# IONIQ6000/av1-go

Measured on AMD Instinct MI355X. Metric: encoded 4K30 frames/sec (whole node) at fixed QP; PSNR-Y delta vs libaom, higher is better.
Workload: dtype u16

## Files before the change

av1-go_amd/csrc/av1_ops32.hpp:

```cpp
#pragma once
#include "av1_ops.hpp"

namespace av1ops {

enum SlotK32 : int {
  K_SKIP = 0,
  K_PART32 = 1,
  K_PART64 = 2,
  K_USE_WIENER = 3,
  K_TXB_SKIP_Y = 4,
  K_TXB_SKIP_C = 5,
  K_EOB_Y = 8,
  K_EOB_C = 9,
  K_EOBX_Y = 10,
  K_EOBX_C = 19,
  K_DC_SIGN_Y = 26,
  K_DC_SIGN_C = 29,
  K_BASE_EOB_Y = 32,
  K_BASE_EOB_C = 36,
  K_BASE_Y = 40,
  K_BASE_C = 66,
  K_BR_Y = 92,
  K_BR_C = 113,
  K_KF_Y_MODE = 134,
  K_UV_MODE = 159,
  K_ANGLE = 172,
  K_END = 180
};
static_assert((int)K_END <= (int)S_MAX, "the slot arrays of the coder are sized by S_MAX");

constexpr BandSlots kSlots32 = { K_USE_WIENER, K_KF_Y_MODE, K_UV_MODE, K_ANGLE, K_TXB_SKIP_Y, K_TXB_SKIP_C, K_EOB_Y, K_EOB_C, K_EOBX_Y, K_EOBX_C,
                                 K_DC_SIGN_Y, K_DC_SIGN_C, K_BASE_EOB_Y, K_BASE_EOB_C, K_BASE_Y, K_BASE_C, K_BR_Y, K_BR_C, 11, 9 };

AV1_HD int slot_nsym_k32(int s) {
  if (const int n = coeff_nsym<kSlots32>(s)) return n;
  if (s == K_SKIP || s == K_USE_WIENER) return 2;
  if (s < K_KF_Y_MODE) return 10;
  if (s < K_UV_MODE) return 13;
  if (s < K_ANGLE) return 14;
  return 7;
}

template <int N> AV1_HD int scan_index32(int pos) {
  const int r = pos / N, c = pos % N, d = r + c;
  const int before = d < N ? d * (d + 1) / 2 : N * N - (2 * N - 1 - d) * (2 * N - d) / 2;
  const int rmin = imax(0, d - N + 1), rmax = imin(d, N - 1);
  return before + ((d & 1) ? r - rmin : rmax - r);
}
struct ScanTables32 { uint16_t s32[1024]; uint8_t s16[256]; };
AV1_HD void fill_scan_tables32(ScanTables32 *t, int tid = 0, int nthreads = 1) {
  for (int pos = tid; pos < 1024; pos += nthreads) t->s32[scan_index32<32>(pos)] = (uint16_t)pos;
  for (int pos = tid; pos < 256; pos += nthreads) t->s16[scan_index32<16>(pos)] = (uint8_t)pos;
}
enum { kMag32Stride = 36 };
template <int N> struct Mag32 { enum { kNibbleBytes = (N + 2) * kMag32Stride / 2, kBytes = kNibbleBytes + N * N / 8 }; };
static_assert(Mag32<32>::kBytes % 4 == 0 && Mag32<16>::kBytes % 4 == 0, "maps follow each other on dwords");
struct TokScratch32 { uint8_t *mag; const ScanTables32 *scan; };

#if defined(__HIP_DEVICE_COMPILE__)
#define AV1_SHARED_ADD(p, v) atomicAdd(p, v)
#define AV1_SHARED_MAX(p, v) atomicMax(p, v)
#else
#define AV1_SHARED_ADD(p, v) (*(p) += (v))
#define AV1_SHARED_MAX(p, v) (*(p) = *(p) > (v) ? *(p) : (v))
#endif

template <int N> struct MagMap<N, false> {
  enum { LG = N == 16 ? 4 : 5, MS = kMag32Stride };
  uint8_t *mag, *sgn;
  const ScanTables32 *scan;
  AV1_HD MagMap(const TokScratch32 &ts) : mag(ts.mag), sgn(ts.mag + Mag32<N>::kNibbleBytes), scan(ts.scan) {}
  AV1_HD int load8(const int16_t *lev, int r, int *cul) {
    struct alignas(16) L8 { int16_t v[8]; } q = *reinterpret_cast<const L8 *>(lev + 8 * r);
    unsigned packed = 0, signs = 0;
    int eob = 0, sum = 0;
    for (int j = 0; j < 8; j++) {
      const int v = q.v[j], a = iabs(v);
      if (v) eob = imax(eob, scan_index32<N>(8 * r + j) + 1);
      sum += a;
      packed |= (unsigned)(a > 15 ? 15 : a) << (4 * j);
      signs |= (unsigned)(v < 0) << j;
    }
    if (!sum) return 0;
    const int at = (((8 * r) >> LG) * MS + ((8 * r) & (N - 1))) >> 1;
    *reinterpret_cast<u16a *>(mag + at) = (uint16_t)packed;
    *reinterpret_cast<u16a *>(mag + at + 2) = (uint16_t)(packed >> 16);
    sgn[r] = (uint8_t)signs;
    *cul += sum;
    return eob;
  }
  AV1_HD int pos(int c) const { return N == 16 ? (int)scan->s16[c] : (int)scan->s32[c]; }
  AV1_HD int at(int i) const { return (mag[i >> 1] >> ((i & 1) << 2)) & 15; }
  AV1_HD int neg(int p) const { return (sgn[p >> 3] >> (p & 7)) & 1; }
};

enum { kLanes32 = 64, kBlocks32 = 4, kTile32MagBytes = kBlocks32 * (Mag32<32>::kBytes + 2 * Mag32<16>::kBytes) };
template <class T, int kStore> struct LaneVar {
  T v[kStore];
  AV1_HD T &operator[](int lane) { return v[kStore == 1 ? 0 : lane]; }
};
enum { kRoundSlots = 4 + 26 + 21, kRoundStride = 33 };
AV1_HD int round_slot(int slot, bool chroma) {
  const int be = chroma ? K_BASE_EOB_C : K_BASE_EOB_Y, ba = chroma ? K_BASE_C : K_BASE_Y, br = chroma ? K_BR_C : K_BR_Y;
  return slot >= br ? 30 + slot - br : slot >= ba ? 4 + slot - ba : slot - be;
}
AV1_HD int round_slot_global(int rs, bool chroma) {
  const int be = chroma ? K_BASE_EOB_C : K_BASE_EOB_Y, ba = chroma ? K_BASE_C : K_BASE_Y, br = chroma ? K_BR_C : K_BR_Y;
  return rs >= 30 ? br + rs - 30 : rs >= 4 ? ba + rs - 4 : be + rs;
}
struct RoundCounts { uint32_t w[kLanes32 / 4]; };

struct Tile32Mem {
  ScanTables32 scan;
  alignas(16) uint8_t mag[kTile32MagBytes];
  uint32_t round[kRoundSlots * kRoundStride];
  uint32_t run[K_END];
  int eob[kBlocks32 * 3], cul[kBlocks32 * 3];
};
AV1_HD TokScratch32 tile_scratch32(Tile32Mem &S, int b, int p) {
  return { S.mag + b * (Mag32<32>::kBytes + 2 * Mag32<16>::kBytes) + (p ? Mag32<32>::kBytes + (p - 1) * Mag32<16>::kBytes : 0), &S.scan };
}

AV1_HD int lit_words(int nbits) { return (nbits + 10) / 11; }
template <class F> AV1_HD void lit_pieces(unsigned v, int nbits, F put) {
  while (nbits > 11) { nbits -= 11; put(op_lit(11, (v >> nbits) & 0x7FFu)); }
  if (nbits > 0) put(op_lit(nbits, v & ((1u << nbits) - 1u)));
}
struct WordSink32 {
  int n;
  AV1_HD void sym(int, int) { n++; }
  AV1_HD void lit(unsigned, int nbits) { n += lit_words(nbits); }
};
struct TotalSink32 {
  uint32_t *tot; int n;
  AV1_HD void sym(int slot, int) { AV1_SHARED_ADD(&tot[slot], 1u); n++; }
  AV1_HD void split(int, int slot) { sym(slot, 0); }
  AV1_HD void lit(unsigned, int nbits) { n += lit_words(nbits); }
};
struct CountSink32 {
  uint8_t *col; bool chroma; int n;
  AV1_HD void sym(int slot, int) { col[round_slot(slot, chroma) * (kRoundStride * 4)]++; n++; }
  AV1_HD void lit(unsigned, int nbits) { n += lit_words(nbits); }
};
struct EmitSink32 {
  u16a *col; bool chroma; int n; op_t *list; uint32_t *grouped;
  AV1_HD void sym(int slot, int s) { u16a &p = col[round_slot(slot, chroma) * (kRoundStride * 2)]; grouped[p] = ((uint32_t)n << 4) | (uint32_t)s; p++; n++; }
  AV1_HD void lit(unsigned v, int nbits) { lit_pieces(v, nbits, [&](op_t o) { list[n++] = o; }); }
};
struct DirectSink32 {
  uint32_t *run; int n; op_t *list; uint32_t *grouped;
  AV1_HD void sym(int slot, int s) { grouped[run[slot]++] = ((uint32_t)n << 4) | (uint32_t)s; n++; }
  AV1_HD void split(int kind, int slot) { sym(slot, kind ? kSplitVert : kSplitHorz); }
  AV1_HD void lit(unsigned v, int nbits) { lit_pieces(v, nbits, [&](op_t o) { list[n++] = o; }); }
};

AV1_HD long block_index32(const FrameView &f, int sbr, int sbc, int b) { return (long)(sbr * 2 + (b >> 1)) * (f.w8 / 4) + sbc * 2 + (b & 1); }

template <class K> AV1_HD void tok_block32_head(const FrameView &f, K &k, int sbr, int sbc, int b, bool half) {
  const int w32 = f.w8 / 4, by = b >> 1, bx = b & 1;
  const long i = block_index32(f, sbr, sbc, b);
  if (b == 0) {
    tok_lr<kSlots32>(f, k, sbr, sbc);
    if (half) k.split(1, K_PART64);
    else k.sym(K_PART64, 3);
  }
  k.sym(K_PART32, 0);
  k.sym(K_SKIP, 0);
  tok_kf_modes<kSlots32>(k, f.y_mode[i], f.uv_mode[i], by ? f.y_mode[i - w32] : 0, bx ? f.y_mode[i - 1] : 0);
}
AV1_HD void tile_sum32(Tile32Mem &S, int b, int p, int *cul, int *dc) {
  const TokScratch32 ts = tile_scratch32(S, b, p);
  *cul = imin(S.cul[b * 3 + p], 63);
  *dc = (ts.mag[0] & 15) ? ((ts.mag[p ? (int)Mag32<16>::kNibbleBytes : (int)Mag32<32>::kNibbleBytes] & 1) ? 1 : 2) : 0;
}
struct TbCtx32 { int ac, ad, lc, ld; };
AV1_HD TbCtx32 tile_ctx32(Tile32Mem &S, int b, int p) {
  TbCtx32 c = { 0, 0, 0, 0 };
  if (b >> 1) tile_sum32(S, b - 2, p, &c.ac, &c.ad);
  if (b & 1) tile_sum32(S, b - 1, p, &c.lc, &c.ld);
  return c;
}
template <int N, class K> AV1_HD void tok_tb32_open(const FrameView &f, K &k, Tile32Mem &S, int sbr, int sbc, int b, int p, bool half) {
  if (p == 0) tok_block32_head(f, k, sbr, sbc, b, half);
  const TbCtx32 c = tile_ctx32(S, b, p);
  tok_coeffs_lead<N, kSlots32>(k, p != 0, S.eob[b * 3 + p], c.ac, c.ad, c.lc, c.ld, -1, 0);
}
AV1_HD const int16_t *tile_levels32(const FrameView &f, long i, int p) { return p == 0 ? f.lev_y + i * 1024 : (p == 1 ? f.lev_u : f.lev_v) + i * 256; }
template <int N> struct Range32 {
  enum { kRange = N * N / kLanes32 };
  AV1_HD static int count(int eob) { return (eob + kRange - 1) / kRange; }
  template <class K> AV1_HD static void pass1(K &k, Tile32Mem &S, const int16_t *lev, int b, int p, int eob, int ri) {
    const MagMap<N> M(tile_scratch32(S, b, p));
    tok_coeffs_pass1<N, kSlots32>(k, M, p != 0, lev, eob, imin(eob, (ri + 1) * kRange) - 1, ri * kRange);
  }
  template <class K> AV1_HD static void pass2(K &k, Tile32Mem &S, const int16_t *lev, int b, int p, int eob, int ri) {
    const MagMap<N> M(tile_scratch32(S, b, p));
    const TbCtx32 c = ri == 0 ? tile_ctx32(S, b, p) : TbCtx32{ 0, 0, 0, 0 };
    tok_coeffs_pass2<N, kSlots32>(k, M, p != 0, lev, c.ad, c.ld, ri * kRange, imin(eob, (ri + 1) * kRange));
  }
};

template <int N> AV1_HD void tok_tb32_total(const FrameView &f, TotalSink32 &k, Tile32Mem &S, int lane, int sbr, int sbc, int b, int p, bool half) {
  const int eob = S.eob[b * 3 + p];
  const int16_t *lev = tile_levels32(f, block_index32(f, sbr, sbc, b), p);
  if (lane == 0) tok_tb32_open<N>(f, k, S, sbr, sbc, b, p, half);
  if (lane < Range32<N>::count(eob)) { Range32<N>::pass1(k, S, lev, b, p, eob, lane); Range32<N>::pass2(k, S, lev, b, p, eob, lane); }
}

template <int N, class W>
AV1_HD int tok_tb32_emit(W &w, Tile32Mem &S, const FrameView &f, int sbr, int sbc, int b, int p, bool half, int words, op_t *list, uint32_t *grouped) {
  typedef typename W::template Var<int> LaneInt;
  typedef Range32<N> R;
  const int eob = S.eob[b * 3 + p], nr = R::count(eob);
  const int16_t *lev = tile_levels32(f, block_index32(f, sbr, sbc, b), p);
  const bool chroma = p != 0;
  LaneInt n, opened;
  if (nr <= 1) {
    w.each([&](int lane) {
      if (lane) return;
      DirectSink32 k = { S.run, words, list, grouped };
      tok_tb32_open<N>(f, k, S, sbr, sbc, b, p, half);
      if (nr) { R::pass1(k, S, lev, b, p, eob, 0); R::pass2(k, S, lev, b, p, eob, 0); }
      n[lane] = k.n;
    });
    return w.first(n);
  }
  w.each([&](int lane) {
    int c = 0, o = 0;
    if (lane == 0) {
      DirectSink32 k = { S.run, words, list, grouped };
      tok_tb32_open<N>(f, k, S, sbr, sbc, b, p, half);
      o = k.n - words;
    }
    if (lane < ((nr + 3) & ~3)) {
      uint8_t *col = reinterpret_cast<uint8_t *>(S.round) + lane;
      for (int rs = 0; rs < kRoundSlots; rs++) col[rs * (kRoundStride * 4)] = 0;
      if (lane < nr) {
        CountSink32 k = { col, chroma, 0 };
        R::pass1(k, S, lev, b, p, eob, nr - 1 - lane);
        c = k.n;
      }
    }
    opened[lane] = o; n[lane] = c + o;
  });
  const int words1 = w.scan(n);
  typename W::template Var<RoundCounts> cnt;
  const int nd = (nr + 3) >> 2;
  w.each([&](int lane) {
    if (lane >= kRoundSlots) return;
    RoundCounts &c = cnt[lane];
    AV1_UNROLL
    for (int q = 0; q < kLanes32 / 4; q++) c.w[q] = q < nd ? S.round[lane * kRoundStride + q] : 0u;
  });
  w.each([&](int lane) {
    if (lane >= kRoundSlots) return;
    const RoundCounts &c = cnt[lane];
    const int slot = round_slot_global(lane, chroma);
    uint32_t run = S.run[slot];
    AV1_UNROLL
    for (int q = 0; q < kLanes32 / 4; q++) {
      if (q >= nd) continue;
      const uint32_t u = c.w[q], p0 = run, p1 = p0 + (u & 0xFF), p2 = p1 + ((u >> 8) & 0xFF), p3 = p2 + ((u >> 16) & 0xFF);
      run = p3 + (u >> 24);
      S.round[lane * kRoundStride + 2 * q] = p0 | (p1 << 16); S.round[lane * kRoundStride + 2 * q + 1] = p2 | (p3 << 16);
    }
    S.run[slot] = run;
  });
  w.each([&](int lane) {
    if (lane >= nr) return;
    EmitSink32 k = { reinterpret_cast<u16a *>(S.round) + lane, chroma, words + n[lane] + opened[lane], list, grouped };
    R::pass1(k, S, lev, b, p, eob, nr - 1 - lane);
  });
  words += words1;
  w.each([&](int lane) {
    WordSink32 k = { 0 };
    if (lane < nr) R::pass2(k, S, lev, b, p, eob, lane);
    n[lane] = k.n;
  });
  const int words2 = w.scan(n);
  w.each([&](int lane) {
    if (lane >= nr) return;
    DirectSink32 k = { S.run, words + n[lane], list, grouped };
    R::pass2(k, S, lev, b, p, eob, lane);
  });
  return words + words2;
}

struct CallerAreas {
  op_t *list_; uint32_t *grouped_; uint16_t *slot_total, *slot_base;
  AV1_HD void reserve(int, int, int *a, int *b) const { *a = 0; *b = 0; }
  AV1_HD op_t *list(int) const { return list_; }
  AV1_HD uint32_t *grouped(int) const { return grouped_; }
  AV1_HD void slot(int sl, uint16_t total, uint16_t base) const { slot_total[sl] = total; slot_base[sl] = base; }
  AV1_HD void refuse(int sl) const { slot_total[sl] = 0; }
};

template <class W, class O>
AV1_HD int tok_tile32(W &w, Tile32Mem &S, const FrameView &f, int sbr, int sbc, uint32_t ops_cap, O &out) {
  typedef typename W::template Var<int> LaneInt;
  const bool half = sbc * 8 + 4 >= f.w8;
  w.each([&](int lane) {
    fill_scan_tables32(&S.scan, lane, kLanes32);
    for (int i = lane; i < kTile32MagBytes / 4; i += kLanes32) reinterpret_cast<u32a *>(S.mag)[i] = 0;
    for (int i = lane; i < K_END; i += kLanes32) S.run[i] = 0;
    if (lane < kBlocks32 * 3) { S.eob[lane] = 0; S.cul[lane] = 0; }
  });
  w.each([&](int lane) {
    AV1_UNROLL
    for (int b = 0; b < kBlocks32; b++) {
      if (half && (b & 1)) continue;
      const long i = block_index32(f, sbr, sbc, b);
      int eob = 0, cul = 0;
      MagMap<32> Y(tile_scratch32(S, b, 0));
      eob = Y.load8(f.lev_y + i * 1024, lane, &cul);
      eob = imax(eob, Y.load8(f.lev_y + i * 1024, lane + kLanes32, &cul));
      if (cul) { AV1_SHARED_MAX(&S.eob[b * 3], eob); AV1_SHARED_ADD(&S.cul[b * 3], cul); }
      const int p = 1 + (lane >> 5);
      MagMap<16> C(tile_scratch32(S, b, p));
      cul = 0;
      eob = C.load8((p == 1 ? f.lev_u : f.lev_v) + i * 256, lane & 31, &cul);
      if (cul) { AV1_SHARED_MAX(&S.eob[b * 3 + p], eob); AV1_SHARED_ADD(&S.cul[b * 3 + p], cul); }
    }
  });
  LaneInt n;
  w.each([&](int lane) {
    TotalSink32 k = { S.run, 0 };
    for (int b = 0; b < kBlocks32; b++) {
      if (half && (b & 1)) continue;
      tok_tb32_total<32>(f, k, S, lane, sbr, sbc, b, 0, half);
      tok_tb32_total<16>(f, k, S, lane, sbr, sbc, b, 1, half);
      tok_tb32_total<16>(f, k, S, lane, sbr, sbc, b, 2, half);
    }
    n[lane] = k.n;
  });
  const int words = w.scan(n);
  enum { kOwn = (K_END + kLanes32 - 1) / kLanes32 };
  w.each([&](int lane) {
    int mine = 0;
    for (int q = 0; q < kOwn; q++) if (lane * kOwn + q < K_END) mine += (int)((S.run[lane * kOwn + q] + kListAlign - 1) & ~(uint32_t)(kListAlign - 1));
    n[lane] = mine;
  });
  const int entries = w.scan(n);
  const bool fits = (uint32_t)words <= ops_cap && entries <= 65535;
  w.each([&](int lane) {
    uint32_t run = (uint32_t)n[lane];
    for (int q = 0; q < kOwn; q++) {
      const int sl = lane * kOwn + q;
      if (sl >= K_END) break;
      const uint32_t tot = S.run[sl];
      out.slot(sl, (uint16_t)(fits ? tot : 0u), (uint16_t)(fits ? run : 0u));
      S.run[sl] = run;
      run += (tot + kListAlign - 1) & ~(uint32_t)(kListAlign - 1);
    }
    for (int sl = K_END + lane; sl < S_MAX; sl += kLanes32) out.slot(sl, 0, 0);
  });
  if (!fits) return -1;
  LaneInt at_list, at_grouped;
  w.each([&](int lane) { if (lane == 0) out.reserve(words, entries, &at_list[lane], &at_grouped[lane]); });
  op_t *const list = out.list(w.first(at_list));
  uint32_t *const grouped = out.grouped(w.first(at_grouped));
  int at = 0;
  for (int b = 0; b < kBlocks32; b++) {
    if (half && (b & 1)) continue;
    at = tok_tb32_emit<32>(w, S, f, sbr, sbc, b, 0, half, at, list, grouped);
    at = tok_tb32_emit<16>(w, S, f, sbr, sbc, b, 1, half, at, list, grouped);
    at = tok_tb32_emit<16>(w, S, f, sbr, sbc, b, 2, half, at, list, grouped);
  }
  return at;
}

}
```

Before: 3288.

## Tokenize all transform blocks of a 64x64 tile in parallel lane groups

Replaces the per-transform-block sequential emit (each block doing its own count, scan and emit phases across the wave) with a schedule that assigns lane groups to all luma blocks at once and then to all chroma blocks, so the coefficient passes of several blocks run concurrently. Per-block heads, including the DC sign context, are emitted serially by one lane, and per-block offsets are tracked in new at1/at2 arrays. Round counters move from 8-bit to 16-bit columns, which drops the packed-byte prefix step. This cuts the number of wave-wide barrier phases per tile, at the cost of more complex offset bookkeeping and a serial single-lane head pass. A host self-test checks that the output does not depend on lane order.

```diff
diff --git a/av1-go_amd/csrc/av1_ops32.hpp b/av1-go_amd/csrc/av1_ops32.hpp
--- a/av1-go_amd/csrc/av1_ops32.hpp
+++ b/av1-go_amd/csrc/av1_ops32.hpp
@@ -108,7 +108,6 @@
   const int be = chroma ? K_BASE_EOB_C : K_BASE_EOB_Y, ba = chroma ? K_BASE_C : K_BASE_Y, br = chroma ? K_BR_C : K_BR_Y;
   return rs >= 30 ? br + rs - 30 : rs >= 4 ? ba + rs - 4 : be + rs;
 }
-struct RoundCounts { uint32_t w[kLanes32 / 4]; };
 
 struct Tile32Mem {
   ScanTables32 scan;
@@ -116,6 +115,7 @@
   uint32_t round[kRoundSlots * kRoundStride];
   uint32_t run[K_END];
   int eob[kBlocks32 * 3], cul[kBlocks32 * 3];
+  int at1[kBlocks32 * 3], at2[kBlocks32 * 3];
 };
 AV1_HD TokScratch32 tile_scratch32(Tile32Mem &S, int b, int p) {
   return { S.mag + b * (Mag32<32>::kBytes + 2 * Mag32<16>::kBytes) + (p ? Mag32<32>::kBytes + (p - 1) * Mag32<16>::kBytes : 0), &S.scan };
@@ -138,14 +138,24 @@
   AV1_HD void lit(unsigned, int nbits) { n += lit_words(nbits); }
 };
 struct CountSink32 {
-  uint8_t *col; bool chroma; int n;
-  AV1_HD void sym(int slot, int) { col[round_slot(slot, chroma) * (kRoundStride * 4)]++; n++; }
+  u16a *col; bool chroma; int n;
+  AV1_HD void sym(int slot, int) { col[round_slot(slot, chroma) * (kRoundStride * 2)]++; n++; }
   AV1_HD void lit(unsigned, int nbits) { n += lit_words(nbits); }
 };
 struct EmitSink32 {
-  u16a *col; bool chroma; int n; op_t *list; uint32_t *grouped;
-  AV1_HD void sym(int slot, int s) { u16a &p = col[round_slot(slot, chroma) * (kRoundStride * 2)]; grouped[p] = ((uint32_t)n << 4) | (uint32_t)s; p++; n++; }
+  u16a *col; const uint32_t *base; bool chroma; int n; op_t *list; uint32_t *grouped;
+  AV1_HD void sym(int slot, int s) { u16a &p = col[round_slot(slot, chroma) * (kRoundStride * 2)]; grouped[base[slot] + p] = ((uint32_t)n << 4) | (uint32_t)s; p++; n++; }
   AV1_HD void lit(unsigned v, int nbits) { lit_pieces(v, nbits, [&](op_t o) { list[n++] = o; }); }
+};
+struct LitSink32 {
+  int n; op_t *list;
+  AV1_HD void sym(int, int) { n++; }
+  AV1_HD void lit(unsigned v, int nbits) { lit_pieces(v, nbits, [&](op_t o) { list[n++] = o; }); }
+};
+struct SignSink32 {
+  uint32_t *run; int n; uint32_t *grouped;
+  AV1_HD void sym(int slot, int s) { grouped[run[slot]++] = ((uint32_t)n << 4) | (uint32_t)s; n++; }
+  AV1_HD void lit(unsigned, int nbits) { n += lit_words(nbits); }
 };
 struct DirectSink32 {
   uint32_t *run; int n; op_t *list; uint32_t *grouped;
@@ -186,104 +196,111 @@
   tok_coeffs_lead<N, kSlots32>(k, p != 0, S.eob[b * 3 + p], c.ac, c.ad, c.lc, c.ld, -1, 0);
 }
 AV1_HD const int16_t *tile_levels32(const FrameView &f, long i, int p) { return p == 0 ? f.lev_y + i * 1024 : (p == 1 ? f.lev_u : f.lev_v) + i * 256; }
-template <int N> struct Range32 {
-  enum { kRange = N * N / kLanes32 };
-  AV1_HD static int count(int eob) { return (eob + kRange - 1) / kRange; }
-  template <class K> AV1_HD static void pass1(K &k, Tile32Mem &S, const int16_t *lev, int b, int p, int eob, int ri) {
+
+template <bool kChroma> struct Step32 {
+  enum { N = kChroma ? 16 : 32, kGroupLanes = kChroma ? 8 : 16 };
+  int tb, b, p, j;
+  int eob, per, nr;
+  const int16_t *lev;
+  AV1_HD Step32(const Tile32Mem &S, const FrameView &f, int sbr, int sbc, int lane) {
+    const int g = lane / kGroupLanes;
+    j = lane % kGroupLanes;
+    b = kChroma ? g >> 1 : g; p = kChroma ? 1 + (g & 1) : 0; tb = b * 3 + p;
+    eob = S.eob[tb];
+    per = (eob + kGroupLanes - 1) / kGroupLanes;
+    nr = eob ? (eob + per - 1) / per : 0;
+    lev = j < nr ? tile_levels32(f, block_index32(f, sbr, sbc, b), p) : nullptr;
+  }
+  template <class K> AV1_HD void pass1(K &k, Tile32Mem &S) const {
     const MagMap<N> M(tile_scratch32(S, b, p));
-    tok_coeffs_pass1<N, kSlots32>(k, M, p != 0, lev, eob, imin(eob, (ri + 1) * kRange) - 1, ri * kRange);
-  }
-  template <class K> AV1_HD static void pass2(K &k, Tile32Mem &S, const int16_t *lev, int b, int p, int eob, int ri) {
+    const int r = nr - 1 - j;
+    tok_coeffs_pass1<N, kSlots32>(k, M, kChroma, lev, eob, imin(eob, (r + 1) * per) - 1, r * per);
+  }
+  template <class K> AV1_HD void pass2(K &k, Tile32Mem &S) const {
     const MagMap<N> M(tile_scratch32(S, b, p));
-    const TbCtx32 c = ri == 0 ? tile_ctx32(S, b, p) : TbCtx32{ 0, 0, 0, 0 };
-    tok_coeffs_pass2<N, kSlots32>(k, M, p != 0, lev, c.ad, c.ld, ri * kRange, imin(eob, (ri + 1) * kRange));
-  }
-};
-
-template <int N> AV1_HD void tok_tb32_total(const FrameView &f, TotalSink32 &k, Tile32Mem &S, int lane, int sbr, int sbc, int b, int p, bool half) {
-  const int eob = S.eob[b * 3 + p];
-  const int16_t *lev = tile_levels32(f, block_index32(f, sbr, sbc, b), p);
-  if (lane == 0) tok_tb32_open<N>(f, k, S, sbr, sbc, b, p, half);
-  if (lane < Range32<N>::count(eob)) { Range32<N>::pass1(k, S, lev, b, p, eob, lane); Range32<N>::pass2(k, S, lev, b, p, eob, lane); }
-}
-
-template <int N, class W>
-AV1_HD int tok_tb32_emit(W &w, Tile32Mem &S, const FrameView &f, int sbr, int sbc, int b, int p, bool half, int words, op_t *list, uint32_t *grouped) {
-  typedef typename W::template Var<int> LaneInt;
-  typedef Range32<N> R;
-  const int eob = S.eob[b * 3 + p], nr = R::count(eob);
-  const int16_t *lev = tile_levels32(f, block_index32(f, sbr, sbc, b), p);
-  const bool chroma = p != 0;
-  LaneInt n, opened;
-  if (nr <= 1) {
-    w.each([&](int lane) {
-      if (lane) return;
-      DirectSink32 k = { S.run, words, list, grouped };
-      tok_tb32_open<N>(f, k, S, sbr, sbc, b, p, half);
-      if (nr) { R::pass1(k, S, lev, b, p, eob, 0); R::pass2(k, S, lev, b, p, eob, 0); }
-      n[lane] = k.n;
-    });
-    return w.first(n);
-  }
-  w.each([&](int lane) {
-    int c = 0, o = 0;
-    if (lane == 0) {
-      DirectSink32 k = { S.run, words, list, grouped };
-      tok_tb32_open<N>(f, k, S, sbr, sbc, b, p, half);
-      o = k.n - words;
-    }
-    if (lane < ((nr + 3) & ~3)) {
-      uint8_t *col = reinterpret_cast<uint8_t *>(S.round) + lane;
-      for (int rs = 0; rs < kRoundSlots; rs++) col[rs * (kRoundStride * 4)] = 0;
-      if (lane < nr) {
-        CountSink32 k = { col, chroma, 0 };
-        R::pass1(k, S, lev, b, p, eob, nr - 1 - lane);
-        c = k.n;
+    tok_coeffs_pass2<N, kSlots32>(k, M, kChroma, lev, 0, 0, j * per, imin(eob, (j + 1) * per));
+  }
+};
+
+template <bool kChroma, bool kFirst, class W, class V>
+AV1_HD void tok_step32_count(W &w, Tile32Mem &S, const FrameView &f, int sbr, int sbc, V &n1, V &n2) {
+  w.each([&](int lane) {
+    const Step32<kChroma> st(S, f, sbr, sbc, lane);
+    u16a *col = reinterpret_cast<u16a *>(S.round) + lane;
+    AV1_UNROLL
+    for (int rs = 0; rs < kRoundSlots; rs++) col[rs * (kRoundStride * 2)] = 0;
+    int c1 = 0, c2 = 0;
+    if (st.j < st.nr) {
+      CountSink32 k = { col, kChroma, 0 };
+      st.pass1(k, S);
+      c1 = k.n;
+      if (kFirst) {
+        WordSink32 k2 = { 0 };
+        st.pass2(k2, S);
+        c2 = k2.n;
+        AV1_SHARED_ADD(&S.at1[st.tb], c1); AV1_SHARED_ADD(&S.at2[st.tb], c2);
       }
     }
-    opened[lane] = o; n[lane] = c + o;
-  });
-  const int words1 = w.scan(n);
-  typename W::template Var<RoundCounts> cnt;
-  const int nd = (nr + 3) >> 2;
+    if (kFirst) { n1[lane] = c1; n2[lane] = c2; }
+  });
   w.each([&](int lane) {
     if (lane >= kRoundSlots) return;
-    RoundCounts &c = cnt[lane];
+    u32a *row = reinterpret_cast<u32a *>(S.round) + lane * kRoundStride;
+    uint32_t run = 0;
     AV1_UNROLL
-    for (int q = 0; q < kLanes32 / 4; q++) c.w[q] = q < nd ? S.round[lane * kRoundStride + q] : 0u;
-  });
-  w.each([&](int lane) {
-    if (lane >= kRoundSlots) return;
-    const RoundCounts &c = cnt[lane];
-    const int slot = round_slot_global(lane, chroma);
-    uint32_t run = S.run[slot];
-    AV1_UNROLL
-    for (int q = 0; q < kLanes32 / 4; q++) {
-      if (q >= nd) continue;
-      const uint32_t u = c.w[q], p0 = run, p1 = p0 + (u & 0xFF), p2 = p1 + ((u >> 8) & 0xFF), p3 = p2 + ((u >> 16) & 0xFF);
-      run = p3 + (u >> 24);
-      S.round[lane * kRoundStride + 2 * q] = p0 | (p1 << 16); S.round[lane * kRoundStride + 2 * q + 1] = p2 | (p3 << 16);
-    }
-    S.run[slot] = run;
-  });
-  w.each([&](int lane) {
-    if (lane >= nr) return;
-    EmitSink32 k = { reinterpret_cast<u16a *>(S.round) + lane, chroma, words + n[lane] + opened[lane], list, grouped };
-    R::pass1(k, S, lev, b, p, eob, nr - 1 - lane);
-  });
-  words += words1;
-  w.each([&](int lane) {
-    WordSink32 k = { 0 };
-    if (lane < nr) R::pass2(k, S, lev, b, p, eob, lane);
-    n[lane] = k.n;
-  });
-  const int words2 = w.scan(n);
-  w.each([&](int lane) {
-    if (lane >= nr) return;
-    DirectSink32 k = { S.run, words + n[lane], list, grouped };
-    R::pass2(k, S, lev, b, p, eob, lane);
-  });
-  return words + words2;
+    for (int q = 0; q < kLanes32 / 2; q++) {
+      const uint32_t u = row[q], p0 = run, p1 = p0 + (u & 0xFFFFu);
+      run = p1 + (u >> 16);
+      row[q] = (p0 & 0xFFFFu) | (p1 << 16);
+    }
+    if (kFirst) S.run[round_slot_global(lane, kChroma)] = run;
+  });
+}
+template <bool kChroma, class W, class V>
+AV1_HD void tok_step32_write(W &w, Tile32Mem &S, const FrameView &f, int sbr, int sbc, V &x1, V &x2, op_t *list, uint32_t *grouped) {
+  w.each([&](int lane) {
+    const Step32<kChroma> st(S, f, sbr, sbc, lane);
+    if (st.j >= st.nr) return;
+    EmitSink32 k = { reinterpret_cast<u16a *>(S.round) + lane, S.run, kChroma, S.at1[st.tb] + x1[lane], list, grouped };
+    st.pass1(k, S);
+    LitSink32 k2 = { S.at2[st.tb] + x2[lane], list };
+    st.pass2(k2, S);
+  });
+}
+template <int N> AV1_HD int tok_tb32_head(Tile32Mem &S, const FrameView &f, int sbr, int sbc, int b, int p, bool half, int at, int *before1, int *before2,
+                                          op_t *list, uint32_t *grouped) {
+  const int tb = b * 3 + p, c1 = S.at1[tb], c2 = S.at2[tb];
+  DirectSink32 k = { S.run, at, list, grouped };
+  tok_tb32_open<N>(f, k, S, sbr, sbc, b, p, half);
+  S.at1[tb] = k.n - *before1; S.at2[tb] = k.n + c1 - *before2;
+  *before1 += c1; *before2 += c2;
+  if (S.eob[tb]) {
+    SignSink32 s = { S.run, k.n + c1, grouped };
+    const MagMap<N> M(tile_scratch32(S, b, p));
+    const TbCtx32 c = tile_ctx32(S, b, p);
+    tok_coeffs_pass2<N, kSlots32>(s, M, p != 0, tile_levels32(f, block_index32(f, sbr, sbc, b), p), c.ad, c.ld, 0, 1);
+  }
+  return k.n + c1 + c2;
+}
+template <int N> AV1_HD int tok_tb32_head_total(Tile32Mem &S, const FrameView &f, int sbr, int sbc, int b, int p, bool half) {
+  TotalSink32 k = { S.run, 0 };
+  tok_tb32_open<N>(f, k, S, sbr, sbc, b, p, half);
+  if (S.eob[b * 3 + p]) {
+    TotalSink32 s = { S.run, 0 };
+    const MagMap<N> M(tile_scratch32(S, b, p));
+    const TbCtx32 c = tile_ctx32(S, b, p);
+    tok_coeffs_pass2<N, kSlots32>(s, M, p != 0, tile_levels32(f, block_index32(f, sbr, sbc, b), p), c.ad, c.ld, 0, 1);
+  }
+  return k.n;
+}
+AV1_HD void tok_tile32_heads(Tile32Mem &S, const FrameView &f, int sbr, int sbc, bool half, op_t *list, uint32_t *grouped) {
+  int at = 0, y1 = 0, y2 = 0, c1 = 0, c2 = 0;
+  for (int b = 0; b < kBlocks32; b++) {
+    if (half && (b & 1)) continue;
+    at = tok_tb32_head<32>(S, f, sbr, sbc, b, 0, half, at, &y1, &y2, list, grouped);
+    at = tok_tb32_head<16>(S, f, sbr, sbc, b, 1, half, at, &c1, &c2, list, grouped);
+    at = tok_tb32_head<16>(S, f, sbr, sbc, b, 2, half, at, &c1, &c2, list, grouped);
+  }
 }
 
 struct CallerAreas {
@@ -303,7 +320,7 @@
     fill_scan_tables32(&S.scan, lane, kLanes32);
     for (int i = lane; i < kTile32MagBytes / 4; i += kLanes32) reinterpret_cast<u32a *>(S.mag)[i] = 0;
     for (int i = lane; i < K_END; i += kLanes32) S.run[i] = 0;
-    if (lane < kBlocks32 * 3) { S.eob[lane] = 0; S.cul[lane] = 0; }
+    if (lane < kBlocks32 * 3) { S.eob[lane] = 0; S.cul[lane] = 0; S.at1[lane] = 0; S.at2[lane] = 0; }
   });
   w.each([&](int lane) {
     AV1_UNROLL
@@ -322,16 +339,14 @@
       if (cul) { AV1_SHARED_MAX(&S.eob[b * 3 + p], eob); AV1_SHARED_ADD(&S.cul[b * 3 + p], cul); }
     }
   });
-  LaneInt n;
-  w.each([&](int lane) {
-    TotalSink32 k = { S.run, 0 };
-    for (int b = 0; b < kBlocks32; b++) {
-      if (half && (b & 1)) continue;
-      tok_tb32_total<32>(f, k, S, lane, sbr, sbc, b, 0, half);
-      tok_tb32_total<16>(f, k, S, lane, sbr, sbc, b, 1, half);
-      tok_tb32_total<16>(f, k, S, lane, sbr, sbc, b, 2, half);
-    }
-    n[lane] = k.n;
+  LaneInt y1, y2, c1, c2, n;
+  tok_step32_count<true, true>(w, S, f, sbr, sbc, c1, c2);
+  tok_step32_count<false, true>(w, S, f, sbr, sbc, y1, y2);
+  w.each([&](int lane) {
+    const int b = lane / 3, p = lane - b * 3;
+    int head = 0;
+    if (lane < kBlocks32 * 3 && !(half && (b & 1))) head = p == 0 ? tok_tb32_head_total<32>(S, f, sbr, sbc, b, p, half) : tok_tb32_head_total<16>(S, f, sbr, sbc, b, p, half);
+    n[lane] = head + y1[lane] + y2[lane] + c1[lane] + c2[lane];
   });
   const int words = w.scan(n);
   enum { kOwn = (K_END + kLanes32 - 1) / kLanes32 };
@@ -359,14 +374,12 @@
   w.each([&](int lane) { if (lane == 0) out.reserve(words, entries, &at_list[lane], &at_grouped[lane]); });
   op_t *const list = out.list(w.first(at_list));
   uint32_t *const grouped = out.grouped(w.first(at_grouped));
-  int at = 0;
-  for (int b = 0; b < kBlocks32; b++) {
-    if (half && (b & 1)) continue;
-    at = tok_tb32_emit<32>(w, S, f, sbr, sbc, b, 0, half, at, list, grouped);
-    at = tok_tb32_emit<16>(w, S, f, sbr, sbc, b, 1, half, at, list, grouped);
-    at = tok_tb32_emit<16>(w, S, f, sbr, sbc, b, 2, half, at, list, grouped);
-  }
-  return at;
-}
-
-}
+  w.scan(y1); w.scan(y2); w.scan(c1); w.scan(c2);
+  w.each([&](int lane) { if (lane == 0) tok_tile32_heads(S, f, sbr, sbc, half, list, grouped); });
+  tok_step32_write<false>(w, S, f, sbr, sbc, y1, y2, list, grouped);
+  tok_step32_count<true, false>(w, S, f, sbr, sbc, c1, c2);
+  tok_step32_write<true>(w, S, f, sbr, sbc, c1, c2, list, grouped);
+  return words;
+}
+
+}
diff --git a/av1-go_amd/host/tok32_selftest.cpp b/av1-go_amd/host/tok32_selftest.cpp
--- /dev/null
+++ b/av1-go_amd/host/tok32_selftest.cpp
@@ -0,0 +1,103 @@
+#include <cstdint>
+#include <cstdio>
+#include <cstdlib>
+#include <cstring>
+#include <vector>
+
+#include "../csrc/av1_ops32.hpp"
+
+using namespace av1ops;
+
+template <bool kDescending> struct WaveLoop {
+  template <class T> using Var = LaneVar<T, kLanes32>;
+  template <class F> void each(F f) { for (int i = 0; i < kLanes32; i++) f(kDescending ? kLanes32 - 1 - i : i); }
+  int scan(Var<int> &v) {
+    int run = 0;
+    for (int lane = 0; lane < kLanes32; lane++) { const int x = v.v[lane]; v.v[lane] = run; run += x; }
+    return run;
+  }
+  int first(Var<int> &v) { return v.v[0]; }
+};
+
+static uint32_t rnd_state = 1;
+static uint32_t rnd() { rnd_state = rnd_state * 1664525u + 1013904223u; return rnd_state >> 8; }
+
+static void fill_block(int16_t *a, int n, const ScanTables32 &scan, int eob, int lo, int hi) {
+  memset(a, 0, sizeof(int16_t) * n * n);
+  auto pos = [&](int c) { return n == 32 ? (int)scan.s32[c] : (int)scan.s16[c]; };
+  if (eob < 0) {
+    for (int i = 0; i < n * n; i++) a[i] = (int16_t)((lo + (int)(rnd() % (uint32_t)(hi - lo + 1))) * ((rnd() & 1) ? -1 : 1));
+    return;
+  }
+  for (int c = 0; c < eob; c++) if (rnd() % 5 < 3) a[pos(c)] = (int16_t)((1 + (int)(rnd() % 4)) * ((rnd() & 1) ? -1 : 1));
+  if (eob) a[pos(eob - 1)] = (rnd() & 1) ? 3 : -1;
+  if (eob > 2) { a[pos(0)] = (int16_t)(15 + rnd() % 3000); a[pos(2)] = (int16_t)-(int)(15 + rnd() % 3000); }
+}
+
+struct Areas {
+  std::vector<uint32_t> list, grouped;
+  std::vector<uint16_t> total, base;
+  Areas(size_t words, size_t entries) : list(words, 0xA5A5A5A5u), grouped(entries, 0xA5A5A5A5u), total(S_MAX, 0x5A5A), base(S_MAX, 0x5A5A) {}
+  CallerAreas out() { return { list.data(), grouped.data(), total.data(), base.data() }; }
+  size_t used() const { size_t e = 0; for (int s = 0; s < S_MAX; s++) if (total[s] && (size_t)base[s] + total[s] > e) e = (size_t)base[s] + total[s]; return e; }
+};
+
+static int fail(const char *what, int c, int w, int h, int sbr, int sbc) {
+  fprintf(stderr, "tok32_selftest: case %d at %dx%d, tile (%d, %d): %s\n", c, w, h, sbr, sbc, what);
+  return 1;
+}
+
+int main() {
+  ScanTables32 scan;
+  fill_scan_tables32(&scan);
+  static const int kEobY[4] = { 1024, 17, 300, 7 }, kEobU[4] = { 256, 3, 0, 100 }, kEobV[4] = { 9, 256, 8, 0 }, kSizes[3][2] = { { 64, 64 }, { 128, 64 }, { 64, 128 } };
+  std::vector<Tile32Mem> mem(1);
+  int tiles = 0;
+  for (int c = 0; c < 6; c++) for (const auto &wh : kSizes) {
+    const int w = wh[0], h = wh[1], w32 = w / 32, nblk = w32 * (h / 32);
+    std::vector<uint8_t> ym(nblk), uvm(nblk);
+    std::vector<int16_t> ly((size_t)nblk * 1024), lu((size_t)nblk * 256), lv((size_t)nblk * 256);
+    for (int i = 0; i < nblk; i++) {
+      const int b = ((i / w32) & 1) * 2 + ((i % w32) & 1);
+      ym[i] = (uint8_t)(rnd() % 13); uvm[i] = (uint8_t)(rnd() % 13);
+      int16_t *y = &ly[(size_t)i * 1024], *u = &lu[(size_t)i * 256], *v = &lv[(size_t)i * 256];
+      switch (c) {
+        case 0: fill_block(y, 32, scan, 0, 0, 0); fill_block(u, 16, scan, kEobU[b] ? kEobU[b] : 5, 0, 0); fill_block(v, 16, scan, 64, 0, 0); break;
+        case 1: fill_block(y, 32, scan, b == 3 ? 700 : 0, 0, 0); fill_block(u, 16, scan, b == 3 ? 90 : 0, 0, 0); fill_block(v, 16, scan, b == 3 ? 256 : 0, 0, 0); break;
+        case 2: fill_block(y, 32, scan, -1, 1, 3000); fill_block(u, 16, scan, -1, 1, 3000); fill_block(v, 16, scan, -1, 1, 3000); break;
+        case 3: fill_block(y, 32, scan, -1, 15, 400); fill_block(u, 16, scan, -1, 15, 400); fill_block(v, 16, scan, -1, 15, 400); break;
+        case 4: fill_block(y, 32, scan, 1, 0, 0); fill_block(u, 16, scan, 1, 0, 0); fill_block(v, 16, scan, 1, 0, 0); break;
+        default: fill_block(y, 32, scan, kEobY[b], 0, 0); fill_block(u, 16, scan, kEobU[b], 0, 0); fill_block(v, 16, scan, kEobV[b], 0, 0); break;
+      }
+    }
+    FrameView f;
+    memset(&f, 0, sizeof(f));
+    f.w8 = w / 8; f.h8 = h / 8; f.key = 1;
+    f.y_mode = ym.data(); f.uv_mode = uvm.data(); f.lev_y = ly.data(); f.lev_u = lu.data(); f.lev_v = lv.data();
+    for (int sbr = 0; sbr < h / 64; sbr++) for (int sbc = 0; sbc < w / 64; sbc++, tiles++) {
+      Areas big(1u << 17, (1u << 17) + 4 * S_MAX);
+      WaveLoop<false> up;
+      CallerAreas o1 = big.out();
+      const int n = tok_tile32(up, mem[0], f, sbr, sbc, 1u << 17, o1);
+      if (n <= 0) return fail("not coded", c, w, h, sbr, sbc);
+      const size_t entries = big.used();
+      Areas exact((size_t)n, entries);
+      WaveLoop<true> down;
+      CallerAreas o2 = exact.out();
+      if (tok_tile32(down, mem[0], f, sbr, sbc, (uint32_t)n, o2) != n) return fail("the lanes in descending order give another length", c, w, h, sbr, sbc);
+      if (exact.total != big.total || exact.base != big.base) return fail("the lanes in descending order give other totals or bases", c, w, h, sbr, sbc);
+      if (memcmp(exact.list.data(), big.list.data(), sizeof(uint32_t) * (size_t)n) || memcmp(exact.grouped.data(), big.grouped.data(), sizeof(uint32_t) * entries))
+        return fail("the lanes in descending order give other words or entries", c, w, h, sbr, sbc);
+      for (int s = 0; s < S_MAX; s++) for (int i = 1; i < big.total[s]; i++)
+        if ((big.grouped[big.base[s] + i] >> 4) <= (big.grouped[big.base[s] + i - 1] >> 4)) return fail("a slot's entries out of decoding order", c, w, h, sbr, sbc);
+      Areas none((size_t)n, entries);
+      CallerAreas o3 = none.out();
+      if (tok_tile32(down, mem[0], f, sbr, sbc, (uint32_t)n - 1, o3) != -1) return fail("a tile one word past the capacity is not refused", c, w, h, sbr, sbc);
+      for (uint32_t x : none.list) if (x != 0xA5A5A5A5u) return fail("a refused tile wrote a list word", c, w, h, sbr, sbc);
+      for (uint32_t x : none.grouped) if (x != 0xA5A5A5A5u) return fail("a refused tile wrote an entry", c, w, h, sbr, sbc);
+      for (uint16_t x : none.total) if (x) return fail("a refused tile has a slot total", c, w, h, sbr, sbc);
+    }
+  }
+  printf("tok32_selftest OK: %d tiles, the lanes of a phase in both orders\n", tiles);
+  return 0;
+}
```

Measured after the change: 3325, median of 6. 1.01x the previous value.
